# YuemingJin/STswinCL

Measured on AMD Instinct MI355X. Metric: input frames/s, TswinPlus fwd+bwd+Adam, 4-frame 512x512 clips, higher is better.
Workload: dtype bf16; 1 GPU; BASELINE.json configs[1]: TswinPlus(12) seg train step, 4 clips/GPU x T=4 frames x 3x512x512, swin res (64,64), OHEM-CE, Adam; T=4 because the reference asserts it (swin_512.py:313); clips_per_gpu=4, frames_per_clip=4, parallelism=dp1, graph_requested=True

## Files before the change

include/stswin_hip.h:

```cpp
#ifndef STSWIN_HIP_H
#define STSWIN_HIP_H
#ifdef __cplusplus
extern "C" {
#endif

#define STSWIN_GF_GELU 1
#define STSWIN_GF_RESID 2
#define STSWIN_GF_MUL_DGELU 4
#define STSWIN_GF_OUT_F32 8
#define STSWIN_GF_ACCUM 16
#define STSWIN_GF_RELU 32
#define STSWIN_GF_MUL_R 8192
#define STSWIN_GF_C2_DGELU 16384
#define STSWIN_GF_CS_PARTIAL 32768
#define STSWIN_GF_CS_SQ 65536
#define STSWIN_GF_TAPSKIP (1 << 29)
#define STSWIN_GF_BIG 128
#define STSWIN_GF_MID 512
#define STSWIN_GF_NOPIPE 1024
#define STSWIN_GF_HALF 2048
#define STSWIN_GF_M32PP (1u << 31)
#define STSWIN_GF_W4R (1 << 30)
#define STSWIN_GF_ROT 4096
#define STSWIN_GF_NOBIG 256
// ... 33 lines not shown
                        int W, int Ho, int Wo, int C, int backward, void* stream);
int stswin_conv3x3_c64(const void* x, const void* wmat, void* y, const void* resid, float* stats, int frames, int H, int W, int sign,
                       void* stream);
long stswin_conv3x3_c64_wgrad_scratch(int frames, int H, int W);
int stswin_conv3x3_c64_wgrad(const void* dy, const void* x, float* dw, int tapminor, int accumulate, float* scratch, long scratch_floats,
                             int frames, int H, int W, void* stream);

int stswin_gemm_nt(int dtype, const void* A, long lda, const int* a_rows, const void* B, long ldb, void* C, long ldc,
                   const int* c_rows, void* C2, long ldc2, const float* bias, const void* R, long ldr,
                   const int* r_rows, int M, int N, int Kseg, int S, float scale, int scale_cols, int flags,
                   float* colsum , void* stream);
int stswin_cs_reduce(const float* partials, int M, int N, float* out, void* stream);
#define STSWIN_TN_OVERWRITE (1 << 27)
#define STSWIN_TN_NO_COMBINE (1 << 26)
long stswin_gemm_nt_splitk_scratch(int M, int N, int Kseg, int S);
int stswin_gemm_nt_splitk(const void* A, long lda, const int* a_rows, const void* B, long ldb, void* C, long ldc, const float* bias, int M, int N,
                          int Kseg, int S, int relu, float* workspace, long workspace_floats, void* stream);
int stswin_tn_fused_hold(int delta);
int stswin_set_cu_budget(int cus);
int stswin_gemm_tn(int dtype, const void* At, long lda, const int* at_rows, const void* Bt, long ldb, const int* bt_rows,
                   float* C, long ldc, int Mk, int Ni, int Nj, int splits, int bseg,
                   float* workspace , long workspace_floats, void* stream);
#define STSWIN_TN_GROUP_DECLINED (-1050)
typedef struct stswin_tn_problem {
  const void* At; long lda; const int* at_rows;
  const void* Bt; long ldb; const int* bt_rows;
  float* C; long ldc;
  int Mk, Ni, Nj, bseg;
  int overwrite;
  int tapminor;
} stswin_tn_problem;
int stswin_gemm_tn_group(int dtype, int count, const stswin_tn_problem* problems, float* workspace, long workspace_floats, int* splits_out,
                         void* stream);
int stswin_tn_combine(const float* workspace, float* C, long ldc, int Ni, int Nj, int splits, int overwrite, int slab_bf16,
                      void* stream);
#define STSWIN_VAR_F32 100
#define STSWIN_VAR_NT_RING256_REGEPI 1
#define STSWIN_VAR_NT_RING256_LDSEPI 2
#define STSWIN_VAR_NT_RING256_NOPIPE 3
#define STSWIN_VAR_NT_RING256_W4 14
#define STSWIN_VAR_NT_STREAM 4
#define STSWIN_VAR_NT_DUO 5
#define STSWIN_VAR_NT_RING256x128_PP 6
#define STSWIN_VAR_NT_MID 7
#define STSWIN_VAR_NT_256x64 8
#define STSWIN_VAR_NT_128x64 9
#define STSWIN_VAR_NT_128x128 10
#define STSWIN_VAR_NT_128x128_W4 11
#define STSWIN_VAR_NT_SPLITK 13
#define STSWIN_VAR_NT_ROWS 12
#define STSWIN_VAR_TN_RING_PLAIN 20
#define STSWIN_VAR_TN_RING_ATROWS 21
#define STSWIN_VAR_TN_RING_BTROWS 22
#define STSWIN_VAR_TN_RING_BSEG 23
#define STSWIN_VAR_TN_128x128 30
#define STSWIN_VAR_TN_128x128_W4 31
#define STSWIN_VAR_TN_ROWS 32
#define STSWIN_VAR_TN_SLABS_F32 0x1000
#define STSWIN_VAR_TN_SLABS_BF16 0x2000
#define STSWIN_VAR_TN_FUSED 0x8000
#define STSWIN_VAR_TN_TAPMINOR 0x4000
#define STSWIN_TN_OUT_TAPMINOR (1 << 25)
int stswin_gemm_nt_qkv_fp8(const void* A, long lda, const int* a_rows, const void* B, long ldb, void* out8, long ld8, float* scales,
                           long ld_scales, const float* bias, int M, int N, int Kseg, float scale, int scale_cols, int rows_per_problem,
                           int head_dim, void* stream);
int stswin_win_attn_fwd_f8(const void* qkv8, long ld8, const float* scales, long ld_scales, void* out, long ldo, const float* biasT,
// ... 201 lines not shown
```

stswincl_amd/csrc/gemm.hip:

```cpp
#include "common.h"
#include "stswin_hip.h"
#include <cstdint>
#include <cstdlib>
#include <type_traits>

enum {
  GF_GELU = STSWIN_GF_GELU, GF_RESID = STSWIN_GF_RESID, GF_MUL_DGELU = STSWIN_GF_MUL_DGELU, GF_OUT_F32 = STSWIN_GF_OUT_F32,
  GF_ACCUM = STSWIN_GF_ACCUM, GF_RELU = STSWIN_GF_RELU, GF_MUL_R = STSWIN_GF_MUL_R, GF_C2_DGELU = STSWIN_GF_C2_DGELU,
  GF_CS_PARTIAL = STSWIN_GF_CS_PARTIAL, GF_CS_SQ = STSWIN_GF_CS_SQ, GF_TAPSKIP = STSWIN_GF_TAPSKIP,
  GF_WAVES4 = STSWIN_GF_WAVES4, GF_BIG = STSWIN_GF_BIG, GF_NOBIG = STSWIN_GF_NOBIG, GF_MID = STSWIN_GF_MID, GF_NOPIPE = STSWIN_GF_NOPIPE,
  GF_HALF = STSWIN_GF_HALF, GF_ROT = STSWIN_GF_ROT, GF_NOREGEPI = STSWIN_GF_NOREGEPI, GF_NOSTREAM = STSWIN_GF_NOSTREAM,
  GF_DUO = STSWIN_GF_DUO, GF_STREAM = STSWIN_GF_STREAM, GF_NONARROW = STSWIN_GF_NONARROW, GF_NODEEP = STSWIN_GF_NODEEP,
  GF_DEEP = STSWIN_GF_DEEP, GF_W4R = STSWIN_GF_W4R, GF_M32PP = (int)STSWIN_GF_M32PP,
};

#ifdef STSWIN_TUNING
#define STSWIN_DBG(flags, bit) (((flags) & (1 << (bit))) != 0)
#else
#define STSWIN_DBG(flags, bit) false
#endif
enum { GF_DEBUG_BITS = (1 << 17) | (1 << 18) | (1 << 19) | (1 << 20) | (1 << 21) };
#ifdef STSWIN_TUNING
static __device__ int g_dbg_stagger[2] = {8, 0};
extern "C" int stswin_debug_set_stagger(int phases, int ticks) {
// ... 1016 lines not shown
      mma_all();
      if (!lag && kt + 1 < nt) wait_tile(kt + 1);
    }
    if (!lag) __builtin_amdgcn_s_barrier();
    if (arow_bad) __builtin_trap();
    if constexpr (SWAP) epilogue_reg();
    else epilogue();
  }
  if constexpr (PERSIST) {
    tix_ += (int)gridDim.x;
    if (tix_ < ntot_) __syncthreads();
  }
  } while (PERSIST && tix_ < ntot_);
}


#ifdef STSWIN_TUNING
#include "gemm_nt_tuning_kernels.inc"
#endif

struct GemmTN {
  const void* At; long lda; const int* at_rows;
  const void* Bt; long ldb; const int* bt_rows;
  float* C; long ldc;
  int Mk, Ni, Nj;
  int splits;
  int bseg;
  float* slabs;
  int slab_bf16;
  unsigned* tile_cnt; int overwrite; int perm;
};

template <typename T, int NW>
__global__ __launch_bounds__(NW * 64) void gemm_tn_kernel(GemmTN p) {
  constexpr int WN = NW / 2, JN = 128 / WN / 16;
  constexpr int PACK = TT<T>::PACK;
  constexpr int BM = TT<T>::IS_BF16 ? 64 : 32;
  constexpr int ROWB = 128 * sizeof(T);
  constexpr int RPI = 1024 / ROWB;
  constexpr int NI = BM / (NW * RPI);
  constexpr int CPR = ROWB / 16;
  extern __shared__ __attribute__((aligned(16))) char smem[];
  const int tid = threadIdx.x, l = tid & 63, w = wave_id();
  const int wr = w / WN, wc = w % WN;
  const int tiles_j = (p.Nj + 127) >> 7;
  const int split_id = blockIdx.x % p.splits, tile_id = blockIdx.x / p.splits;
  const int i0 = (tile_id / tiles_j) << 7, j0 = (tile_id % tiles_j) << 7;
  const int ntile_all = (p.Mk + BM - 1) / BM;
  const int per = (ntile_all + p.splits - 1) / p.splits;
  const int t_begin = split_id * per, t_end = min(ntile_all, t_begin + per);
  if (t_begin >= t_end) return;

  const char* zero = (const char*)g_stswin_zero;
  const int rsub = l / CPR, cphys = l % CPR;
  long arow[NI], brow[NI];
  int bcol[NI];
  bool btap1[NI];
  const int tap0 = p.bseg > 0 ? j0 / p.bseg : 0;
  const int tap1 = p.bseg > 0 ? min(tap0 + 1, p.Nj / p.bseg - 1) : 0;
#pragma unroll
  for (int i = 0; i < NI; ++i) {
    const int r = (w * NI + i) * RPI + rsub;
    const int cj = j0 + ((cphys & ~15) | ((cphys ^ swz256(r)) & 15)) * PACK;
    bcol[i] = p.bseg > 0 ? cj % p.bseg : cj;
    btap1[i] = p.bseg > 0 && cj / p.bseg != tap0;
  }
  typedef int ivec __attribute__((ext_vector_type(RPI)));
  typedef const __attribute__((address_space(4))) ivec* civec;
  const bool vec_maps = (p.Mk % RPI) == 0;
  auto fetch_rows = [&](int tile) {
    const int mw = tile * BM + w * (NI * RPI);
#pragma unroll
    for (int i = 0; i < NI; ++i) {
      const int mb = mw + i * RPI;
      int va[RPI], vb0[RPI], vb1[RPI];
      if (vec_maps && mb + RPI <= p.Mk) {
        ivec ta, t0, t1;
#pragma unroll
        for (int r = 0; r < RPI; ++r) { ta[r] = mb + r; t0[r] = mb + r; t1[r] = -1; }
// ... 89 lines not shown
          const int col = wr * 64 + i * 16 + fr;
          a[i] = *(const float*)(Ab + row * ROWB + ((((col >> 2) & ~15) | (((col >> 2) ^ swz256(row)) & 15)) << 4) + (col & 3) * 4);
        }
#pragma unroll
        for (int j = 0; j < JN; ++j) {
          const int col = wc * (16 * JN) + j * 16 + fr;
          b[j] = *(const float*)(Bb + row * ROWB + ((((col >> 2) & ~15) | (((col >> 2) ^ swz256(row)) & 15)) << 4) + (col & 3) * 4);
        }
#pragma unroll
        for (int i = 0; i < 4; ++i)
#pragma unroll
          for (int j = 0; j < JN; ++j) acc[i][j] = __builtin_amdgcn_mfma_f32_16x16x4f32(a[i], b[j], acc[i][j], 0, 0, 0);
      }
    }
    if (tk + 2 < t_end) fetch_rows(tk + 2);
  }
#pragma unroll
  for (int i = 0; i < 4; ++i)
#pragma unroll
    for (int j = 0; j < JN; ++j)
#pragma unroll
      for (int r = 0; r < 4; ++r) {
        const int gi = i0 + wr * 64 + i * 16 + 4 * fq + r;
        const int gj = j0 + wc * (16 * JN) + j * 16 + fr;
        if (gi < p.Ni && gj < p.Nj) {
          if (p.slabs) {
            const long so = ((long)split_id * p.Ni + gi) * p.Nj + gj;
            if (p.slab_bf16) ((bf16*)p.slabs)[so] = (bf16)acc[i][j][r];
            else p.slabs[so] = acc[i][j][r];
          }
          else atomicAdd(p.C + (long)gi * p.ldc + gj, acc[i][j][r]);
        }
      }
}


#ifdef STSWIN_TUNING
__device__ unsigned long long* g_tn_stamp_buf = nullptr;
extern "C" int stswin_debug_set_tn_stamps(void* buf) { return (int)hipMemcpyToSymbol(HIP_SYMBOL(g_tn_stamp_buf), &buf, sizeof(buf)); }
#endif
template <int MODE, bool FUSE>
DEVI void gemm_tn_ring_body(const GemmTN& p, const int seq, const int nwg, const int stamp_row) {
  constexpr bool MAPS = MODE != 0, MAP_A = MODE == 1, MAP_B = MODE >= 2, TAPS = MODE == 3;
  using T = bf16;
  constexpr int BMK = 32, ROWB = 512, NST = 4, OP_BYTES = BMK * ROWB, STAGE = 2 * OP_BYTES, PER_STAGE = 4;
  constexpr int FI = 8, FJ = 4;
  extern __shared__ __attribute__((aligned(16))) char smem[];
  const int tid = threadIdx.x, l = tid & 63, w = wave_id();
  const int wr = w >> 2, wc = w & 3;
  const int tiles_j = (p.Nj + 255) >> 8;
  const int ntiles_ = nwg / p.splits;
  const int split_id = seq / ntiles_, tile_id = seq - split_id * ntiles_;
  const int i0 = (tile_id / tiles_j) << 8, j0 = (tile_id % tiles_j) << 8;
  const int nst_all = (p.Mk + BMK - 1) / BMK;
  const int per = (nst_all + p.splits - 1) / p.splits;
  const int s_begin = split_id * per, s_end = min(nst_all, s_begin + per);
  const int nt = max(0, s_end - s_begin);
  const bool dbg_ts = p.ldc == -1;
  auto stamp = [&](int slot) {
    if (dbg_ts && threadIdx.x == 0) ((unsigned long long*)p.C)[(long)stamp_row * 8 + slot] = wall_clock64();
#ifdef STSWIN_TUNING
    else if (g_tn_stamp_buf && threadIdx.x == 0) {
      g_tn_stamp_buf[(long)stamp_row * 8 + slot] = wall_clock64();
      if (slot == 0) { g_tn_stamp_buf[(long)stamp_row * 8 + 6] = (unsigned long long)p.Ni; g_tn_stamp_buf[(long)stamp_row * 8 + 7] = (unsigned long long)(split_id * 1000 + tile_id); }
    }
#endif
// ... 304 lines not shown
__global__ __launch_bounds__(512, 2) void gemm_tn_ring_kernel(GemmTN p) {
  gemm_tn_ring_body<MODE, FUSE>(p, xcd_remap((int)blockIdx.x, (int)gridDim.x), (int)gridDim.x, (int)blockIdx.x);
}

#define TN_GROUP_MAX 4
struct GemmTNGroup { GemmTN q[TN_GROUP_MAX]; int first[TN_GROUP_MAX + 1]; int mode[TN_GROUP_MAX]; int count; };
template <int M0, int M1, int M2, int M3>
__global__ __launch_bounds__(512, 2) void gemm_tn_ring_group_static_kernel(GemmTNGroup g) {
  const int seq = xcd_remap((int)blockIdx.x, (int)gridDim.x);
  if constexpr (M3 >= 0) {
    if (seq >= g.first[3]) { gemm_tn_ring_body<M3 < 0 ? 0 : M3, true>(g.q[3], seq - g.first[3], g.first[4] - g.first[3], (int)blockIdx.x); return; }
  }
  if constexpr (M2 >= 0) {
    if (seq >= g.first[2]) { gemm_tn_ring_body<M2 < 0 ? 0 : M2, true>(g.q[2], seq - g.first[2], g.first[3] - g.first[2], (int)blockIdx.x); return; }
  }
  if constexpr (M1 >= 0) {
    if (seq >= g.first[1]) { gemm_tn_ring_body<M1 < 0 ? 0 : M1, true>(g.q[1], seq - g.first[1], g.first[2] - g.first[1], (int)blockIdx.x); return; }
  }
  gemm_tn_ring_body<M0, true>(g.q[0], seq, g.first[1], (int)blockIdx.x);
}
__global__ __launch_bounds__(512, 2) void gemm_tn_ring_group_kernel(GemmTNGroup g) {
  const int seq = xcd_remap((int)blockIdx.x, (int)gridDim.x);
  int i = 0;
  while (i + 1 < g.count && seq >= g.first[i + 1]) ++i;
  const int local = seq - g.first[i], nwg = g.first[i + 1] - g.first[i];
  switch (g.mode[i]) {
    case 0: gemm_tn_ring_body<0, true>(g.q[i], local, nwg, (int)blockIdx.x); break;
    case 1: gemm_tn_ring_body<1, true>(g.q[i], local, nwg, (int)blockIdx.x); break;
    case 2: gemm_tn_ring_body<2, true>(g.q[i], local, nwg, (int)blockIdx.x); break;
    default: gemm_tn_ring_body<3, true>(g.q[i], local, nwg, (int)blockIdx.x); break;
  }
}

__global__ __launch_bounds__(256) void tn_reduce_kernel(const float* slabs, float* C, long ldc, int Ni, int Nj, int splits,
                                                        int overwrite, int slab_bf16, int perm) {
  if (slab_bf16) {
    const long idx = ((long)blockIdx.x * 256 + threadIdx.x) * 8;
    const long total = (long)Ni * Nj;
    if (idx >= total) return;
    const int i = idx / Nj, j = idx % Nj;
    float a[8] = {0.f, 0.f, 0.f, 0.f, 0.f, 0.f, 0.f, 0.f};
    const bf16* src = (const bf16*)slabs + idx;
    int s = 0;
    for (; s + 8 <= splits; s += 8) {
      bf16x8 v[8];
#pragma unroll
      for (int u = 0; u < 8; ++u) v[u] = *(const bf16x8*)(src + (long)(s + u) * total);
#pragma unroll
      for (int u = 0; u < 8; ++u)
#pragma unroll
        for (int e = 0; e < 8; ++e) a[e] += (float)v[u][e];
    }
    for (; s < splits; ++s) {
      const bf16x8 v = *(const bf16x8*)(src + (long)s * total);
#pragma unroll
      for (int e = 0; e < 8; ++e) a[e] += (float)v[e];
    }
    if (perm > 0) {
      const int S = Nj / perm, sg = j / perm, c = j - sg * perm;
      float* d = C + (long)i * ldc + (long)c * S + sg;
#pragma unroll
      for (int e = 0; e < 8; ++e) d[(long)e * S] = overwrite ? a[e] : d[(long)e * S] + a[e];
      return;
    }
    float* dst = C + (long)i * ldc + j;
    if ((ldc & 3) == 0) {
      f32x4 lo = {a[0], a[1], a[2], a[3]}, hi = {a[4], a[5], a[6], a[7]};
      if (!overwrite) { lo += *(const f32x4*)dst; hi += *(const f32x4*)(dst + 4); }
      *(f32x4*)dst = lo;
      *(f32x4*)(dst + 4) = hi;
    } else {
      for (int e = 0; e < 8; ++e) dst[e] = overwrite ? a[e] : dst[e] + a[e];
    }
    return;
  }
  const long idx = ((long)blockIdx.x * 256 + threadIdx.x) * 4;
  if (idx >= (long)Ni * Nj) return;
  const int i = idx / Nj, j = idx % Nj;
  f32x4 a = {0.f, 0.f, 0.f, 0.f};
  for (int s = 0; s < splits; ++s) a += *(const f32x4*)(slabs + (long)s * Ni * Nj + idx);
  if (perm > 0) {
    const int S = Nj / perm, sg = j / perm, c = j - sg * perm;
    float* d = C + (long)i * ldc + (long)c * S + sg;
#pragma unroll
    for (int e = 0; e < 4; ++e) d[(long)e * S] = overwrite ? a[e] : d[(long)e * S] + a[e];
    return;
  }
  float* dst = C + (long)i * ldc + j;
  if (overwrite) {
    if ((ldc & 3) == 0) *(f32x4*)dst = a;
    else { for (int e = 0; e < 4; ++e) dst[e] = a[e]; }
  } else if ((ldc & 3) == 0) { *(f32x4*)dst = *(const f32x4*)dst + a; }
  else { for (int e = 0; e < 4; ++e) dst[e] += a[e]; }
}

static thread_local int g_last_variant[2] = {0, 0};
extern "C" int stswin_tuning_build() {
#ifdef STSWIN_TUNING
  return 1;
#else
  return 0;
#endif
}
extern "C" int stswin_last_variant(int family) { return family >= 0 && family < 2 ? g_last_variant[family] : -1; }

static int set_lds_once(const void* fn) {
  return (int)hipFuncSetAttribute(fn, hipFuncAttributeMaxDynamicSharedMemorySize, 65536);
}

extern "C" int stswin_cs_reduce(const float* partials, int M, int N, float* out, void* stream) {
  if (M <= 0 || N <= 0) return 0;
  if (N % 4) return -1004;
  const int rows = 2 * ((M + 255) / 256);
  const int rc = stswin_fold_launch(partials, N, 0, rows, N, 1, out, nullptr, nullptr, 0, 1, 1, (hipStream_t)stream);
  if (rc) return rc;
  STSWIN_CHECK_LAUNCH();
  return 0;
}

__global__ __launch_bounds__(256) void gemm_nt_rows_kernel(GemmNT p) {
  const int l = threadIdx.x & 63, n = blockIdx.x * 4 + (threadIdx.x >> 6);
  if (n >= p.N) return;
  const bf16* A = (const bf16*)p.A;
  const bf16* Bn = (const bf16*)p.B + (long)n * p.ldb;
  float acc[8] = {0, 0, 0, 0, 0, 0, 0, 0};
  for (int k = l * 8; k < p.Kseg; k += 512) {
// ... 552 lines not shown
  long wo = 0, to = 0;
  for (int i = 0; i < count; ++i) {
    const StswinTnProblem& q = pr[i];
    const int perm = (q.tapminor && q.bseg > 0) ? q.bseg : 0;
    g.q[i] = GemmTN{q.At, q.lda, q.at_rows, q.Bt, q.ldb, q.bt_rows, q.C, q.ldc, q.Mk, q.Ni, q.Nj, rs[i], q.bseg, workspace + wo, 1,
                    cnt + 3 * to, q.overwrite ? 1 : 0, perm};
    g.mode[i] = q.at_rows ? 1 : (q.bt_rows ? (q.bseg > 0 ? 3 : 2) : 0);
    g.first[i + 1] = g.first[i] + tiles[i] * rs[i];
    wo += ((long)rs[i] * q.Ni * q.Nj + 1) / 2 + 64;
    wo = (wo + 63) / 64 * 64;
    to += tiles[i];
    if (splits_out) splits_out[i] = rs[i];
  }
  for (int i = count; i < TN_GROUP_MAX; ++i) { g.q[i] = g.q[0]; g.mode[i] = 0; g.first[i + 1] = g.first[count]; }
  static int once_g = (int)hipFuncSetAttribute((const void*)gemm_tn_ring_group_kernel, hipFuncAttributeMaxDynamicSharedMemorySize, 131072) |
                      (int)hipFuncSetAttribute((const void*)gemm_tn_ring_group_static_kernel<0, 1, 2, -1>, hipFuncAttributeMaxDynamicSharedMemorySize, 131072) |
                      (int)hipFuncSetAttribute((const void*)gemm_tn_ring_group_static_kernel<0, 0, -1, -1>, hipFuncAttributeMaxDynamicSharedMemorySize, 131072) |
                      (int)hipFuncSetAttribute((const void*)gemm_tn_ring_group_static_kernel<0, 0, 1, 2>, hipFuncAttributeMaxDynamicSharedMemorySize, 131072);
  (void)once_g;
  g_last_variant[1] = STSWIN_VAR_TN_RING_PLAIN | STSWIN_VAR_TN_SLABS_BF16 | STSWIN_VAR_TN_FUSED | (rs[0] << 16);
  const bool m012 = count == 3 && g.mode[0] == 0 && g.mode[1] == 1 && g.mode[2] == 2;
  const bool m00 = count == 2 && g.mode[0] == 0 && g.mode[1] == 0;
  const bool m0012 = count == 4 && g.mode[0] == 0 && g.mode[1] == 0 && g.mode[2] == 1 && g.mode[3] == 2;
  static const char* egd = getenv("STSWIN_TN_GROUP_DYNAMIC");
  if (m012 && !(egd && atoi(egd))) hipLaunchKernelGGL((gemm_tn_ring_group_static_kernel<0, 1, 2, -1>), dim3((unsigned)total), dim3(512), 131072, (hipStream_t)stream, g);
  else if (m00 && !(egd && atoi(egd))) hipLaunchKernelGGL((gemm_tn_ring_group_static_kernel<0, 0, -1, -1>), dim3((unsigned)total), dim3(512), 131072, (hipStream_t)stream, g);
  else if (m0012 && !(egd && atoi(egd))) hipLaunchKernelGGL((gemm_tn_ring_group_static_kernel<0, 0, 1, 2>), dim3((unsigned)total), dim3(512), 131072, (hipStream_t)stream, g);
  else
  hipLaunchKernelGGL(gemm_tn_ring_group_kernel, dim3((unsigned)total), dim3(512), 131072, (hipStream_t)stream, g);
  STSWIN_CHECK_LAUNCH();
  return 0;
}

extern "C" int stswin_gemm_tn(int dtype, const void* At, long lda, const int* at_rows, const void* Bt, long ldb,
                              const int* bt_rows, float* C, long ldc, int Mk, int Ni, int Nj, int splits, int bseg,
                              float* workspace, long workspace_floats, void* stream) {
  if (Mk <= 0 || Ni <= 0 || Nj <= 0) return 0;
  const int overwrite = (splits > 0 && (splits & (1 << 27))) ? 1 : 0;
  const int no_combine = (splits > 0 && (splits & (1 << 26))) ? 1 : 0;
  if (splits > 0) splits &= ~(1 << 26);
  const int perm = (splits > 0 && (splits & (1 << 25)) && bseg > 0 && !no_combine) ? bseg : 0;
  if (splits > 0) splits &= ~(1 << 25);
  const char* f32_env = getenv("STSWIN_TN_F32_SLABS");
  const int f32_slabs = f32_env && atoi(f32_env) ? 1 : 0;
  const int slab_bf16 = (dtype == 0 && !f32_slabs) ? 1 : 0;
  if (splits > 0) splits &= ~(1 << 27);
  const int splits_flags_w4 = (splits > 0 && (splits & (1 << 30))) ? 1 : 0;
  if (splits > 0) splits &= ~(1 << 30);
  const int pack = dtype == 0 ? 8 : 4;
  if (Ni % pack || Nj % pack || lda % pack || ldb % pack) return -1003;
  if (bseg < 0 || (bseg > 0 && (bseg % pack || !bt_rows || Nj % bseg))) return -1004;
  if (dtype == 0 && Mk <= 8 && !at_rows && !bt_rows && bseg == 0 && ldc % 4 == 0) {
    g_last_variant[1] = STSWIN_VAR_TN_ROWS;
    const long nthr = (long)Ni * (Nj / 4);
    hipLaunchKernelGGL(gemm_tn_rows_kernel, dim3((unsigned)((nthr + 255) / 256)), dim3(256), 0, (hipStream_t)stream, (const bf16*)At, lda, (const bf16*)Bt,
                       ldb, C, ldc, Mk, Ni, Nj, overwrite);
    STSWIN_CHECK_LAUNCH();
    return 0;
  }
  if (bseg > 0)
    for (int j0 = 0; j0 < Nj; j0 += 128)
      if ((j0 + 127 < Nj ? j0 + 127 : Nj - 1) / bseg - j0 / bseg > 1) return -1005;
  const int bm = dtype == 0 ? 64 : 32;
  const int ntile = (Mk + bm - 1) / bm;
  const bool force_ring = splits > 0 && (splits & (1 << 29));
  const bool no_ring = splits > 0 && (splits & (1 << 28));
// ... 119 lines not shown
```

stswincl_amd/headops.py:

```python
from __future__ import annotations

import os
import weakref
from typing import List, Optional, Sequence, Tuple

import torch
import torch.nn.functional as F

from . import hip
from .ops import compute_dtype, _f32

KGRAN = 64


_INDEX_MAPS = {}
_TORCH_PADVEC = os.environ.get("STSWIN_TORCH_PADVEC") == "1"
_BN_KEEP_Y = os.environ.get("STSWIN_BN_KEEP_Y") == "1"


class Layout:

    def __init__(self, segs: Sequence[Tuple[int, int, int]], width: int):
        self.segs, self.width = list(segs), width
        self.logical = sum(s[1] for s in self.segs)
# ... 136 lines not shown
        tab = hip.stats_table(Mo, lout.width, x.device) if want_stats else None
        ctx.tapskip = hip.GF_TAPSKIP if (k == 3 and stride == 1 and 2 * dil >= Hin + 3 and Mo <= 32768) else 0
        ctx.halo = (_HALO_CONV and bias is None and lin.is_identity and lout.is_identity and X.is_contiguous()
                    and hip.conv3x3_c64_ok(frames, Hin, Win, lin.width, lout.width, k, stride, pad, dil, dt))
        if ctx.halo:
            hip.conv3x3_c64(X, _conv_mats(weight, dt, lin, lout, False), y, frames, Hin, Win, 1, stats_out=tab)
        else:
            hip.gemm_nt(X, _conv_mats(weight, dt, lin, lout, False), y, M=Mo, a_rows=fmap, S=k * k,
                        bias=lout.pad_vec(bias) if bias is not None else None, stats_out=tab, flags=ctx.tapskip)
        ctx.geom = (frames, Hin, Win)
        ctx.cfg = (k, lin, lout, dt, x.dtype, bias is not None, Mi, Mo)
        ctx.save_for_backward(X, weight, fmap, imap)
        if want_stats:
            ctx.mark_non_differentiable(tab)
            ctx.set_materialize_grads(False)
            return y, tab
        return y

    @staticmethod
    @hip.tn_deferred_backward
    def backward(ctx, dy, _dtab=None):
        if dy is None:
            return (None,) * 8
        X, weight, fmap, imap = ctx.saved_tensors
        k, lin, lout, dt, in_dtype, has_bias, Mi, Mo = ctx.cfg
        co, ci = weight.shape[:2]
        S = k * k
        g = dy.detach().to(dt).contiguous()
        from .ops import wgrad_buffer
        dense = lin.is_identity and lout.is_identity
        direct = dense and S == 1
        dwp = (wgrad_buffer(weight, (lout.width, S * lin.width), X.device) if dense
               else torch.empty(lout.width, S * lin.width, dtype=torch.float32, device=X.device))
        if ctx.halo and _HALO_WGRAD and hip.conv3x3_c64_wgrad_ok(*ctx.geom):
            hip.conv3x3_c64_wgrad(g, X, dwp, *ctx.geom, tapminor=True)
            tapminor = True
        else:
            hip.gemm_tn(g, X, dwp, Mk=Mo, bt_rows=fmap, bseg=lin.width if fmap is not None else 0, overwrite=True,
                        tapminor=dense and S > 1)
            tapminor = dense and S > 1 and hip.last_tn_tapminor()
        dx = None
        if ctx.needs_input_grad[0]:
            dx = torch.empty(Mi, lin.width, dtype=dt, device=X.device)
            pend = ctx.link.take(dt, dx.shape) if ctx.link is not None else None
            if ctx.halo:
                hip.conv3x3_c64(g, _conv_mats(weight, dt, lin, lout, True), dx, *ctx.geom, -1, resid=pend)
            else:
                hip.gemm_nt(g, _conv_mats(weight, dt, lin, lout, True), dx, M=Mi, a_rows=imap, S=S, resid=pend,
                            flags=(hip.GF_RESID if pend is not None else 0) | ctx.tapskip)
            dx = dx.to(in_dtype)
            if ctx.link is not None and not ctx.link.last():
                ctx.link.put(dx)
                dx = None
        hip.tn_join()
        if direct or tapminor:
            dw = dwp
        elif dense:
            dw = dwp.clone().view(co, S, ci).permute(0, 2, 1)
        else:
            dw = torch.zeros(co, ci, S, dtype=torch.float32, device=X.device)
            d3 = dwp.view(lout.width, S, lin.width)
            for oa, on, ob in lout.segs:
                for ia, in_, ib in lin.segs:
                    dw[oa:oa + on, ia:ia + in_, :] = d3[ob:ob + on, :, ib:ib + in_].permute(0, 2, 1)
        db = None
        if has_bias:
            dbp = hip.zeros(lout.width, device=X.device)
            hip.colsum(g, dbp)
            db = lout.unpad_vec(dbp)
# ... 757 lines not shown
```

stswincl_amd/hip.py:

```python
from __future__ import annotations

import ctypes
import functools
import os
import re
from typing import Optional

import torch

_ROOT = os.path.dirname(os.path.dirname(os.path.abspath(__file__)))
LIB_PATH = os.environ.get("STSWIN_HIP_LIB") or os.path.join(_ROOT, "stswincl_amd", "lib", "libstswin_hip.so")
HEADER_PATH = os.path.join(_ROOT, "include", "stswin_hip.h")
_lib: Optional[ctypes.CDLL] = None

_c_int, _c_float, _c_void_p = ctypes.c_int, ctypes.c_float, ctypes.c_void_p


class StswinHipError(RuntimeError):
    pass


_C_TYPES = {"int": ctypes.c_int, "long": ctypes.c_long, "float": ctypes.c_float, "double": ctypes.c_double}


def _c_value(name: str, expr: str) -> int:
    tokens = re.findall(r"0[xX][0-9a-fA-F]+|\d+|<<|[-+*()]|\S", re.sub(r"(?<=[0-9a-fA-F])[uU]\b", "", expr))
    if not tokens or not all(re.fullmatch(r"0[xX][0-9a-fA-F]+|\d+|<<|[-+*()]", t) for t in tokens):
        raise StswinHipError(f"{HEADER_PATH}: cannot evaluate `#define STSWIN_{name} {expr.strip()}`")
    try:
        v = int(eval(" ".join(tokens), {"__builtins__": {}}))
    except (SyntaxError, TypeError) as e:
        raise StswinHipError(f"{HEADER_PATH}: cannot evaluate `#define STSWIN_{name} {expr.strip()}`") from e
    return v - (1 << 32) if v >= 1 << 31 else v


@functools.lru_cache(maxsize=None)
def _header():
    with open(HEADER_PATH) as f:
        text = re.sub(r"/\*.*?\*/", "", f.read(), flags=re.S)
    protos = {}
    for ret, name, params in re.findall(r"\b(int|long)\s+(stswin_\w+)\s*\(([^()]*)\)\s*;", text):
        argtypes = []
        for p in ([] if params.strip() == "void" else params.split(",")):
            words = [w for w in p.split() if w != "const"]
            if "*" in p:
                argtypes.append(ctypes.c_void_p)
            elif len(words) == 2 and words[0] in _C_TYPES:
                argtypes.append(_C_TYPES[words[0]])
            else:
                raise StswinHipError(f"{HEADER_PATH}: {name}: cannot bind parameter `{p.strip()}`")
        protos[name] = (_C_TYPES[ret], argtypes)
    unparsed = set(re.findall(r"\b(stswin_\w+)\s*\(", text)) - set(protos)
    if unparsed:
        raise StswinHipError(f"{HEADER_PATH}: cannot bind the declaration of {sorted(unparsed)}")
    consts = {name: _c_value(name, expr) for name, expr in re.findall(r"^[ \t]*#[ \t]*define[ \t]+STSWIN_(\w+)[ \t]+(\S.*)$", text, flags=re.M)}
    return protos, consts


globals().update(_header()[1])


def declared_symbols():
    return sorted(_header()[0])


def load() -> ctypes.CDLL:
    global _lib
    if _lib is not None:
        return _lib
    if not os.path.exists(LIB_PATH):
        raise StswinHipError(f"{LIB_PATH} not found: run `python __graft_entry__.py` (build()) first; "
                             "stswincl_amd has no CPU or eager fallback")
    lib = ctypes.CDLL(LIB_PATH)
    protos = _header()[0]
    missing = [s for s in sorted(protos) if not hasattr(lib, s)]
    if missing and not os.environ.get("STSWIN_HIP_LIB"):
        raise StswinHipError(f"libstswin_hip.so lacks declared symbols: {missing}")
    for s, (restype, argtypes) in protos.items():
        if s not in missing:
            fn = getattr(lib, s)
            fn.restype, fn.argtypes = restype, argtypes
    _lib = lib
    return lib


def tuning_build() -> bool:
    return bool(load().stswin_tuning_build())

# ... 618 lines not shown
def gemm_tn_group(problems) -> bool:
    n = len(problems)
    if n == 0:
        return True
    first = problems[0]["At"]
    if n > 4 or first.dtype != torch.bfloat16 or torch.cuda.is_current_stream_capturing() and first.device not in _TN_WS:
        return False
    arr = (_TnProblem * n)()
    flops = 0.0
    for i, q in enumerate(problems):
        At, Bt, out = q["At"], q["Bt"], q["out"]
        assert out.dtype == torch.float32 and At.dtype == Bt.dtype == torch.bfloat16
        ar, br = q.get("at_rows"), q.get("bt_rows")
        arr[i] = _TnProblem(At.data_ptr(), _ld(At), ar.data_ptr() if ar is not None else None, Bt.data_ptr(), _ld(Bt),
                            br.data_ptr() if br is not None else None, out.data_ptr(), _ld(out), q["Mk"], out.shape[0], out.shape[1],
                            q.get("bseg", 0), 1 if q.get("overwrite", True) else 0, 1 if q.get("tapminor", False) else 0)
        flops += 2.0 * q["Mk"] * out.shape[0] * out.shape[1]
    ws = _tn_workspace(first.device)
    tn_join()
    sp = (_c_int * n)()
    name = "gemm_tn_bf16"
    if _SHAPE_NAMES:
        name += " group " + " + ".join(f"{q['out'].shape[0]}x{q['out'].shape[1]}" for q in problems) + f" Mk={problems[0]['Mk']}"
    with _Span(name, flops) as span:
        rc = load().stswin_gemm_tn_group(0, n, arr, _p(ws), ws.numel(), sp, _stream())
        if rc == TN_GROUP_DECLINED:
            span.cancel()
    if rc == TN_GROUP_DECLINED:
        return False
    _check(rc, "gemm_tn_group")
    LAST_TN_GROUP_SPLITS[:] = list(sp)
    _log_variant("tn_group", (n, problems[0]["Mk"]) + tuple(sp), 1)
    return True


def last_tn_tapminor() -> bool:
    return bool(load().stswin_last_variant(1) & VAR_TN_TAPMINOR)


def last_variant(family: int) -> dict:
    v = load().stswin_last_variant(family)
    return {"kernel": v & 0xFFF, "slabs": "bf16" if v & VAR_TN_SLABS_BF16 else ("f32" if v & VAR_TN_SLABS_F32 else ""),
            "splits": v >> 16}


def vec_gather(v: torch.Tensor, imap: torch.Tensor, fill: float = 0.0) -> torch.Tensor:
    out = torch.empty(imap.numel(), dtype=torch.float32, device=v.device)
    _check(load().stswin_vec_gather(_p(v), _p(imap), _p(out), imap.numel(), fill, _stream()), "vec_gather")
    return out


def vec_gather_multi(vs, imap: torch.Tensor, fills=None, outs=None):
    k, n = len(vs), imap.numel()
    assert 1 <= k <= 4 and all(v.dtype == torch.float32 and v.is_contiguous() for v in vs)
    if outs is None:
        flat = torch.empty(k, (n + 15) // 16 * 16, dtype=torch.float32, device=imap.device)
        outs = [flat[i, :n] for i in range(k)]
    else:
        assert len(outs) == k and all(o.dtype == torch.float32 and o.is_contiguous() and o.numel() == n for o in outs)
    fills = list(fills) if fills is not None else [0.0] * k
    _check(load().stswin_vec_gather_multi(k, (_c_void_p * k)(*[v.data_ptr() for v in vs]), _p(imap), (_c_void_p * k)(*[o.data_ptr() for o in outs]),
                                          n, (_c_float * k)(*[float(f) for f in fills]), _stream()), "vec_gather_multi")
    return outs


def colsum(y: torch.Tensor, out_f32: torch.Tensor, M: Optional[int] = None):
# ... 1036 lines not shown
```

Before: 630.7 frames/s.

## Defer weight-gradient GEMMs and batch them into one multi-problem split-K launch

Weight-gradient TN GEMMs from the head ops are queued during backward instead of run immediately. They are flushed at the end of the autograd graph task as one grouped kernel covering up to 32 problems, followed by a single combine kernel. A planner picks split-K factors per problem so the total tile count fills the GPU, and orders problems longest-first. This targets launch overhead and poor occupancy from many small wgrad GEMMs, at the cost of deferral bookkeeping, an f32 slab workspace, and checks that each parameter's .grad buffer is unchanged.

```diff
diff --git a/include/stswin_hip.h b/include/stswin_hip.h
--- a/include/stswin_hip.h
+++ b/include/stswin_hip.h
@@ -89,6 +89,14 @@
 } stswin_tn_problem;
 int stswin_gemm_tn_group(int dtype, int count, const stswin_tn_problem* problems, float* workspace, long workspace_floats, int* splits_out,
                          void* stream);
+enum {
+  STSWIN_TN_MULTI_FORCE = 1,
+  STSWIN_TN_MULTI_MAX = 32,
+  STSWIN_VAR_TN_MULTI = 33
+};
+long stswin_gemm_tn_multi_scratch(int count, const stswin_tn_problem* problems);
+int stswin_gemm_tn_multi(int dtype, int count, const stswin_tn_problem* problems, float* workspace, long workspace_floats, int* splits_io,
+                         int flags, void* stream);
 int stswin_tn_combine(const float* workspace, float* C, long ldc, int Ni, int Nj, int splits, int overwrite, int slab_bf16,
                       void* stream);
 #define STSWIN_VAR_F32 100
diff --git a/stswincl_amd/csrc/gemm.hip b/stswincl_amd/csrc/gemm.hip
--- a/stswincl_amd/csrc/gemm.hip
+++ b/stswincl_amd/csrc/gemm.hip
@@ -1072,7 +1072,7 @@
 };
 
 template <typename T, int NW>
-__global__ __launch_bounds__(NW * 64) void gemm_tn_kernel(GemmTN p) {
+__device__ __forceinline__ void gemm_tn_tile_body(const GemmTN& p, const int bid) {
   constexpr int WN = NW / 2, JN = 128 / WN / 16;
   constexpr int PACK = TT<T>::PACK;
   constexpr int BM = TT<T>::IS_BF16 ? 64 : 32;
@@ -1084,7 +1084,7 @@
   const int tid = threadIdx.x, l = tid & 63, w = wave_id();
   const int wr = w / WN, wc = w % WN;
   const int tiles_j = (p.Nj + 127) >> 7;
-  const int split_id = blockIdx.x % p.splits, tile_id = blockIdx.x / p.splits;
+  const int split_id = bid % p.splits, tile_id = bid / p.splits;
   const int i0 = (tile_id / tiles_j) << 7, j0 = (tile_id % tiles_j) << 7;
   const int ntile_all = (p.Mk + BM - 1) / BM;
   const int per = (ntile_all + p.splits - 1) / p.splits;
@@ -1240,6 +1240,31 @@
           else atomicAdd(p.C + (long)gi * p.ldc + gj, acc[i][j][r]);
         }
       }
+}
+template <typename T, int NW>
+__global__ __launch_bounds__(NW * 64) void gemm_tn_kernel(GemmTN p) {
+  gemm_tn_tile_body<T, NW>(p, (int)blockIdx.x);
+}
+
+#define TN_MULTI_MAX 32
+struct TnMultiSlot {
+  const void* At; const int* at_rows; const void* Bt; const int* bt_rows; float* C; float* slabs;
+  int lda, ldb, ldc, Mk, Ni, Nj, splits, bseg, overwrite, perm;
+};
+struct GemmTNMulti {
+  TnMultiSlot q[TN_MULTI_MAX];
+  int first[TN_MULTI_MAX + 1];
+  int cfirst[TN_MULTI_MAX + 1];
+  int count;
+};
+static_assert(sizeof(GemmTNMulti) <= 3584, "the problem table must fit the 4 KB kernel argument beside the hidden arguments");
+__global__ __launch_bounds__(512) void gemm_tn_multi_kernel(GemmTNMulti g) {
+  const int bid = (int)blockIdx.x;
+  int i = 0;
+  while (i + 1 < g.count && bid >= g.first[i + 1]) ++i;
+  const TnMultiSlot& s = g.q[i];
+  const GemmTN p{s.At, s.lda, s.at_rows, s.Bt, s.ldb, s.bt_rows, s.C, s.ldc, s.Mk, s.Ni, s.Nj, s.splits, s.bseg, s.slabs, 0, nullptr, 0, 0};
+  gemm_tn_tile_body<bf16, 8>(p, bid - g.first[i]);
 }
 
 
@@ -1610,6 +1635,34 @@
   }
 }
 
+__device__ __forceinline__ void tn_reduce_f32_body(const float* slabs, float* C, long ldc, int Ni, int Nj, int splits, int overwrite, int perm,
+                                                   long blk) {
+  const long idx = (blk * 256 + threadIdx.x) * 4;
+  if (idx >= (long)Ni * Nj) return;
+  const int i = idx / Nj, j = idx % Nj;
+  f32x4 a = {0.f, 0.f, 0.f, 0.f};
+  for (int s = 0; s < splits; ++s) a += *(const f32x4*)(slabs + (long)s * Ni * Nj + idx);
+  if (perm > 0) {
+    const int S = Nj / perm, sg = j / perm, c = j - sg * perm;
+    float* d = C + (long)i * ldc + (long)c * S + sg;
+#pragma unroll
+    for (int e = 0; e < 4; ++e) d[(long)e * S] = overwrite ? a[e] : d[(long)e * S] + a[e];
+    return;
+  }
+  float* dst = C + (long)i * ldc + j;
+  if (overwrite) {
+    if ((ldc & 3) == 0) *(f32x4*)dst = a;
+    else { for (int e = 0; e < 4; ++e) dst[e] = a[e]; }
+  } else if ((ldc & 3) == 0) { *(f32x4*)dst = *(const f32x4*)dst + a; }
+  else { for (int e = 0; e < 4; ++e) dst[e] += a[e]; }
+}
+__global__ __launch_bounds__(256) void tn_multi_combine_kernel(GemmTNMulti g) {
+  const int bid = (int)blockIdx.x;
+  int i = 0;
+  while (i + 1 < g.count && bid >= g.cfirst[i + 1]) ++i;
+  const TnMultiSlot& s = g.q[i];
+  tn_reduce_f32_body(s.slabs, s.C, s.ldc, s.Ni, s.Nj, s.splits, s.overwrite, s.perm, bid - g.cfirst[i]);
+}
 __global__ __launch_bounds__(256) void tn_reduce_kernel(const float* slabs, float* C, long ldc, int Ni, int Nj, int splits,
                                                         int overwrite, int slab_bf16, int perm) {
   if (slab_bf16) {
@@ -1652,24 +1705,7 @@
     }
     return;
   }
-  const long idx = ((long)blockIdx.x * 256 + threadIdx.x) * 4;
-  if (idx >= (long)Ni * Nj) return;
-  const int i = idx / Nj, j = idx % Nj;
-  f32x4 a = {0.f, 0.f, 0.f, 0.f};
-  for (int s = 0; s < splits; ++s) a += *(const f32x4*)(slabs + (long)s * Ni * Nj + idx);
-  if (perm > 0) {
-    const int S = Nj / perm, sg = j / perm, c = j - sg * perm;
-    float* d = C + (long)i * ldc + (long)c * S + sg;
-#pragma unroll
-    for (int e = 0; e < 4; ++e) d[(long)e * S] = overwrite ? a[e] : d[(long)e * S] + a[e];
-    return;
-  }
-  float* dst = C + (long)i * ldc + j;
-  if (overwrite) {
-    if ((ldc & 3) == 0) *(f32x4*)dst = a;
-    else { for (int e = 0; e < 4; ++e) dst[e] = a[e]; }
-  } else if ((ldc & 3) == 0) { *(f32x4*)dst = *(const f32x4*)dst + a; }
-  else { for (int e = 0; e < 4; ++e) dst[e] += a[e]; }
+  tn_reduce_f32_body(slabs, C, ldc, Ni, Nj, splits, overwrite, perm, (long)blockIdx.x);
 }
 
 static thread_local int g_last_variant[2] = {0, 0};
@@ -2288,6 +2324,88 @@
   return 0;
 }
 
+#include "tn_multi_plan.h"
+static int tn_multi_check(int count, const StswinTnProblem* pr, TnMultiPlanIn* in, const int* forced) {
+  for (int i = 0; i < count; ++i) {
+    const StswinTnProblem& q = pr[i];
+    if (q.Mk <= 0 || q.Ni <= 0 || q.Nj <= 0 || !q.At || !q.Bt || !q.C) return -1052;
+    if (q.Ni % 8 || q.Nj % 8 || q.lda % 8 || q.ldb % 8) return -1003;
+    if (q.bseg < 0 || (q.bseg > 0 && (q.bseg % 8 || !q.bt_rows || q.Nj % q.bseg))) return -1004;
+    if (q.bseg > 0)
+      for (int j0 = 0; j0 < q.Nj; j0 += 128)
+        if ((j0 + 127 < q.Nj ? j0 + 127 : q.Nj - 1) / q.bseg - j0 / q.bseg > 1) return -1005;
+    if (q.tapminor && q.bseg <= 0) return -1052;
+    if (q.lda < 0 || q.ldb < 0 || q.ldc < 0 || q.lda > 0x7FFFFFFFL || q.ldb > 0x7FFFFFFFL || q.ldc > 0x7FFFFFFFL) return -1052;
+    if ((long)q.Ni * q.Nj > 0x7FFFFFFFL) return -1052;
+    in[i].tiles = ((q.Ni + 127) / 128) * ((q.Nj + 127) / 128);
+    in[i].ktiles = (q.Mk + 63) / 64;
+    in[i].out_floats = (long)q.Ni * q.Nj;
+    in[i].forced = forced && forced[i] > 0 ? forced[i] : 0;
+  }
+  return 0;
+}
+extern "C" long stswin_gemm_tn_multi_scratch(int count, const StswinTnProblem* pr) {
+  if (count <= 0) return 0;
+  if (count > TN_MULTI_MAX || !pr) return -1052;
+  TnMultiPlanIn in[TN_MULTI_MAX];
+  const int rc = tn_multi_check(count, pr, in, nullptr);
+  if (rc) return rc;
+  int sp[TN_MULTI_MAX], fill_ok = 0;
+  long need = 0;
+  if (tn_multi_plan(count, in, -1, sp, &need, &fill_ok) < 0) return 0;
+  return need;
+}
+extern "C" int stswin_gemm_tn_multi(int dtype, int count, const StswinTnProblem* pr, float* workspace, long workspace_floats, int* splits_io,
+                                    int flags, void* stream) {
+  if (count <= 0) return 0;
+  if (count > TN_MULTI_MAX || !pr) return -1052;
+  const int declined = STSWIN_TN_GROUP_DECLINED;
+  const bool force = (flags & STSWIN_TN_MULTI_FORCE) != 0;
+  TnMultiPlanIn in[TN_MULTI_MAX];
+  const int rc = tn_multi_check(count, pr, in, force ? splits_io : nullptr);
+  if (rc) return rc;
+  if (dtype != 0 || !workspace || workspace_floats <= 0) return declined;
+  { const char* em = getenv("STSWIN_TN_MULTI"); if (em && atoi(em) == 0 && !force) return declined; }
+  int sp[TN_MULTI_MAX], fill_ok = 0;
+  long need = 0;
+  const long total = tn_multi_plan(count, in, workspace_floats, sp, &need, &fill_ok);
+  if (total < 0 || total > 0x3FFFFFFFL || (!fill_ok && !force)) return declined;
+  int order[TN_MULTI_MAX];
+  for (int i = 0; i < count; ++i) order[i] = i;
+  for (int i = 1; i < count; ++i)
+    for (int k = i; k > 0; --k) {
+      const int a = order[k - 1], b = order[k];
+      if ((in[a].ktiles + sp[a] - 1) / sp[a] >= (in[b].ktiles + sp[b] - 1) / sp[b]) break;
+      order[k - 1] = b; order[k] = a;
+    }
+  GemmTNMulti g;
+  g.count = count;
+  g.first[0] = 0;
+  g.cfirst[0] = 0;
+  long wo = 0;
+  for (int k = 0; k < count; ++k) {
+    const int i = order[k];
+    const StswinTnProblem& q = pr[i];
+    g.q[k] = TnMultiSlot{q.At, q.at_rows, q.Bt, q.bt_rows, q.C, workspace + wo, (int)q.lda, (int)q.ldb, (int)q.ldc, q.Mk, q.Ni, q.Nj, sp[i],
+                         q.bseg, q.overwrite ? 1 : 0, (q.tapminor && q.bseg > 0) ? q.bseg : 0};
+    g.first[k + 1] = g.first[k] + in[i].tiles * sp[i];
+    const long cblocks = (in[i].out_floats / 4 + 255) / 256;
+    if (g.cfirst[k] + cblocks > 0x3FFFFFFFL) return declined;
+    g.cfirst[k + 1] = g.cfirst[k] + (int)cblocks;
+    wo += tn_multi_align((long)sp[i] * in[i].out_floats);
+  }
+  for (int k = count; k < TN_MULTI_MAX; ++k) { g.q[k] = g.q[0]; g.first[k + 1] = g.first[count]; g.cfirst[k + 1] = g.cfirst[count]; }
+  if (splits_io)
+    for (int i = 0; i < count; ++i) splits_io[i] = sp[i];
+  static int once_m = set_lds_once((const void*)gemm_tn_multi_kernel);
+  (void)once_m;
+  g_last_variant[1] = STSWIN_VAR_TN_MULTI | STSWIN_VAR_TN_SLABS_F32 | (sp[0] << 16);
+  hipLaunchKernelGGL(gemm_tn_multi_kernel, dim3((unsigned)g.first[count]), dim3(512), 65536, (hipStream_t)stream, g);
+  hipLaunchKernelGGL(tn_multi_combine_kernel, dim3((unsigned)g.cfirst[count]), dim3(256), 0, (hipStream_t)stream, g);
+  STSWIN_CHECK_LAUNCH();
+  return 0;
+}
+
 extern "C" int stswin_gemm_tn(int dtype, const void* At, long lda, const int* at_rows, const void* Bt, long ldb,
                               const int* bt_rows, float* C, long ldc, int Mk, int Ni, int Nj, int splits, int bseg,
                               float* workspace, long workspace_floats, void* stream) {
diff --git a/stswincl_amd/csrc/tn_multi_plan.h b/stswincl_amd/csrc/tn_multi_plan.h
--- /dev/null
+++ b/stswincl_amd/csrc/tn_multi_plan.h
@@ -0,0 +1,72 @@
+#pragma once
+
+#define TN_MULTI_ROUND 512
+#define TN_MULTI_MIN_KTILES 8
+
+struct TnMultiPlanIn {
+  int tiles, ktiles;
+  long out_floats;
+  int forced;
+};
+
+static inline int tn_multi_no_empty(int ktiles, int splits) {
+  if (splits > ktiles) splits = ktiles;
+  if (splits < 1) splits = 1;
+  const int per = (ktiles + splits - 1) / splits;
+  return (ktiles + per - 1) / per;
+}
+
+static inline int tn_multi_splits_for(int ktiles, long target) {
+  long s = target > 0 ? ktiles / target : 1;
+  if (s < 1) s = 1;
+  if (s > ktiles) s = ktiles;
+  for (int guard = 0; guard < 64 && s > 1; ++guard) {
+    if (s >= 8) s &= ~7L;
+    else { long p2 = 1; while (p2 * 2 <= s) p2 *= 2; s = p2; }
+    const int n = tn_multi_no_empty(ktiles, (int)s);
+    const int per = (ktiles + n - 1) / n;
+    const int last = ktiles - (n - 1) * per;
+    if (n == 1 || (per >= TN_MULTI_MIN_KTILES && last >= TN_MULTI_MIN_KTILES)) return n;
+    s = n < s ? n : s - 1;
+  }
+  return 1;
+}
+
+static inline long tn_multi_align(long floats) { return (floats + 63) / 64 * 64; }
+
+static inline long tn_multi_plan(int count, const TnMultiPlanIn* in, long ws_floats, int* splits, long* ws_need, int* fill_ok) {
+  int kmax = TN_MULTI_MIN_KTILES, any_forced = 0;
+  for (int i = 0; i < count; ++i) {
+    if (in[i].ktiles > kmax) kmax = in[i].ktiles;
+    if (in[i].forced > 0) any_forced = 1;
+  }
+  long best_t = -1;
+  double best_cost = 0.0;
+  for (long t = TN_MULTI_MIN_KTILES; t <= kmax; ++t) {
+    long total = 0, need = 0, load = 0, longest = 0, slab = 0;
+    for (int i = 0; i < count; ++i) {
+      const int s = in[i].forced > 0 ? tn_multi_no_empty(in[i].ktiles, in[i].forced) : tn_multi_splits_for(in[i].ktiles, t);
+      const long per = (in[i].ktiles + s - 1) / s;
+      total += (long)in[i].tiles * s;
+      load += (long)in[i].tiles * s * (per + 2);
+      if (per + 2 > longest) longest = per + 2;
+      slab += (long)s * in[i].out_floats;
+      need += tn_multi_align((long)s * in[i].out_floats);
+    }
+    if (ws_floats >= 0 && need > ws_floats) continue;
+    const double gemm = total <= TN_MULTI_ROUND ? (double)longest : (double)load / TN_MULTI_ROUND + 0.5 * (double)longest;
+    const double cost = gemm + (double)slab / 950e3;
+    if (best_t < 0 || cost < best_cost) { best_t = t; best_cost = cost; }
+    if (any_forced) break;
+  }
+  if (best_t < 0) return -1;
+  long total = 0, need = 0;
+  for (int i = 0; i < count; ++i) {
+    splits[i] = in[i].forced > 0 ? tn_multi_no_empty(in[i].ktiles, in[i].forced) : tn_multi_splits_for(in[i].ktiles, best_t);
+    total += (long)in[i].tiles * splits[i];
+    need += tn_multi_align((long)splits[i] * in[i].out_floats);
+  }
+  *ws_need = need;
+  *fill_ok = total * 2 >= TN_MULTI_ROUND;
+  return total;
+}
diff --git a/stswincl_amd/headops.py b/stswincl_amd/headops.py
--- a/stswincl_amd/headops.py
+++ b/stswincl_amd/headops.py
@@ -192,9 +192,13 @@
         direct = dense and S == 1
         dwp = (wgrad_buffer(weight, (lout.width, S * lin.width), X.device) if dense
                else torch.empty(lout.width, S * lin.width, dtype=torch.float32, device=X.device))
+        hip.wgrad_settle(weight)
         if ctx.halo and _HALO_WGRAD and hip.conv3x3_c64_wgrad_ok(*ctx.geom):
             hip.conv3x3_c64_wgrad(g, X, dwp, *ctx.geom, tapminor=True)
             tapminor = True
+        elif (dense and (S == 1 or fmap is not None) and getattr(weight, "_stswin_grad_dest", None) is None
+              and hip.wgrad_defer(weight, g, X, dwp, Mk=Mo, bt_rows=fmap, bseg=lin.width if fmap is not None else 0, tapminor=S > 1)):
+            tapminor = S > 1
         else:
             hip.gemm_tn(g, X, dwp, Mk=Mo, bt_rows=fmap, bseg=lin.width if fmap is not None else 0, overwrite=True,
                         tapminor=dense and S > 1)
diff --git a/stswincl_amd/hip.py b/stswincl_amd/hip.py
--- a/stswincl_amd/hip.py
+++ b/stswincl_amd/hip.py
@@ -54,6 +54,8 @@
     if unparsed:
         raise StswinHipError(f"{HEADER_PATH}: cannot bind the declaration of {sorted(unparsed)}")
     consts = {name: _c_value(name, expr) for name, expr in re.findall(r"^[ \t]*#[ \t]*define[ \t]+STSWIN_(\w+)[ \t]+(\S.*)$", text, flags=re.M)}
+    for body in re.findall(r"\benum\s*\{([^{}]*)\}", text):
+        consts.update({name: _c_value(name, expr) for name, expr in re.findall(r"\bSTSWIN_(\w+)\s*=\s*([^,]+)", body)})
     return protos, consts
 
 
@@ -738,6 +740,144 @@
     LAST_TN_GROUP_SPLITS[:] = list(sp)
     _log_variant("tn_group", (n, problems[0]["Mk"]) + tuple(sp), 1)
     return True
+
+
+LAST_TN_MULTI_SPLITS: list = []
+
+
+def _tn_problem_array(problems):
+    arr = (_TnProblem * len(problems))()
+    flops = 0.0
+    for i, q in enumerate(problems):
+        At, Bt = q["At"], q["Bt"]
+        assert At.dtype == Bt.dtype
+        ar, br = q.get("at_rows"), q.get("bt_rows")
+        if q.get("out") is not None:
+            out = q["out"]
+            assert out.dtype == torch.float32
+            cptr, ldc, (Ni, Nj) = out.data_ptr(), _ld(out), out.shape
+        else:
+            cptr, ldc, (Ni, Nj) = q["out_ptr"], q["ldc"], q["shape"]
+        arr[i] = _TnProblem(At.data_ptr(), _ld(At), ar.data_ptr() if ar is not None else None, Bt.data_ptr(), _ld(Bt),
+                            br.data_ptr() if br is not None else None, cptr, ldc, q["Mk"], Ni, Nj,
+                            q.get("bseg", 0), 1 if q.get("overwrite", True) else 0, 1 if q.get("tapminor", False) else 0)
+        flops += 2.0 * q["Mk"] * Ni * Nj
+    return arr, flops
+
+
+def gemm_tn_multi(problems, splits=None) -> bool:
+    n = len(problems)
+    if n == 0:
+        return True
+    first = problems[0]["At"]
+    if n > TN_MULTI_MAX:
+        raise StswinHipError(f"gemm_tn_multi: {n} problems, at most {TN_MULTI_MAX} per call")
+    if torch.cuda.is_current_stream_capturing() and first.device not in _TN_WS:
+        return False
+    arr, flops = _tn_problem_array(problems)
+    ws = _tn_workspace(first.device)
+    tn_join()
+    sp = (_c_int * n)(*([int(s) for s in splits] if splits is not None else [0] * n))
+    with _Span("gemm_tn_multi_bf16" + (f" n={n}" if _SHAPE_NAMES else ""), flops) as span:
+        rc = load().stswin_gemm_tn_multi(_dt(first), n, arr, _p(ws), ws.numel(), sp, TN_MULTI_FORCE if splits is not None else 0, _stream())
+        if rc == TN_GROUP_DECLINED:
+            span.cancel()
+    if rc == TN_GROUP_DECLINED:
+        return False
+    _check(rc, "gemm_tn_multi")
+    LAST_TN_MULTI_SPLITS[:] = list(sp)
+    _log_variant("tn_multi", (n,) + tuple(sp), 1)
+    return True
+
+
+_WGRAD_QUEUE: list = []
+_WGRAD_TASK = -1
+
+
+def tn_multi_on() -> bool:
+    return os.environ.get("STSWIN_TN_MULTI") != "0"
+
+
+def tn_multi_wants(Mk: int, Ni: int, Nj: int) -> bool:
+    env = os.environ.get("STSWIN_TN_MULTI_MAX_GFLOP")
+    return 2.0 * Mk * Ni * Nj <= (float(env) if env else 24.0) * 1e9
+
+
+def _param_defers(param) -> bool:
+    if param is None or not isinstance(param, torch.Tensor) or not param.is_leaf or param.grad is not None:
+        return False
+    if param._backward_hooks or getattr(param, "_post_accumulate_grad_hooks", None):
+        return False
+    try:
+        return bool(torch._C._will_engine_execute_node(torch.autograd.graph.get_gradient_edge(param).node))
+    except RuntimeError:
+        return False
+
+
+def wgrad_settle(param) -> bool:
+    if not _WGRAD_QUEUE or torch._C._current_graph_task_id() != _WGRAD_TASK:
+        return False
+    mine = [q for q in _WGRAD_QUEUE if q["param"] is param]
+    if not mine:
+        return False
+    _WGRAD_QUEUE[:] = [q for q in _WGRAD_QUEUE if q["param"] is not param]
+    param._stswin_wgrad_shared = True
+    if not gemm_tn_multi(mine, splits=[0] * len(mine)):
+        raise StswinHipError("deferred weight gradient: the library declined an early flush")
+    return True
+
+
+def wgrad_defer(param, At, Bt, out, *, Mk, at_rows=None, bt_rows=None, bseg=0, tapminor=False) -> bool:
+    Ni, Nj = out.shape
+    if wgrad_settle(param) or getattr(param, "_stswin_wgrad_shared", False):
+        return False
+    if not (tn_multi_on() and At.dtype == torch.bfloat16 and Bt.dtype == torch.bfloat16 and tn_multi_wants(Mk, Ni, Nj)
+            and (bseg == 0 or bseg >= 64) and tn_fused_holds() == 0 and _param_defers(param)):
+        return False
+    if torch.cuda.is_current_stream_capturing() and At.device not in _TN_WS:
+        return False
+    global _WGRAD_TASK
+    task = torch._C._current_graph_task_id()
+    if _WGRAD_QUEUE and task != _WGRAD_TASK:
+        del _WGRAD_QUEUE[:]
+    if not _WGRAD_QUEUE:
+        try:
+            torch.autograd.Variable._execution_engine.queue_callback(wgrad_flush)
+        except RuntimeError:
+            return False
+        _WGRAD_TASK = task
+    _WGRAD_QUEUE.append(dict(At=At, Bt=Bt, at_rows=at_rows, bt_rows=bt_rows, Mk=Mk, bseg=bseg, overwrite=True, tapminor=tapminor,
+                             out_ptr=out.data_ptr(), ldc=_ld(out), shape=(Ni, Nj), param=param))
+    return True
+
+
+def wgrad_pending() -> int:
+    return len(_WGRAD_QUEUE)
+
+
+def wgrad_flush():
+    queue = list(_WGRAD_QUEUE)
+    del _WGRAD_QUEUE[:]
+    for q in queue:
+        g = q["param"].grad
+        if g is None or g.data_ptr() != q["out_ptr"]:
+            raise StswinHipError("deferred weight gradient: the .grad of a parameter of shape "
+                                 f"{tuple(q['param'].shape)} is not the buffer the queued GEMM writes ({'None' if g is None else hex(g.data_ptr())} "
+                                 f"against {hex(q['out_ptr'])}): the gradient was cloned or accumulated before it was written")
+    for a in range(0, len(queue), TN_MULTI_MAX):
+        part = queue[a:a + TN_MULTI_MAX]
+        if gemm_tn_multi(part):
+            continue
+        for q in part:
+            Ni, Nj = q["shape"]
+            out = q["param"].grad.view(-1)[:Ni * Nj].view(Ni, Nj) if q["ldc"] == Nj else None
+            if out is None or out.data_ptr() != q["out_ptr"]:
+                raise StswinHipError("deferred weight gradient: cannot rebuild the output view of a declined problem")
+            gemm_tn(q["At"], q["Bt"], out, Mk=q["Mk"], at_rows=q["at_rows"], bt_rows=q["bt_rows"], bseg=q["bseg"], overwrite=True,
+                    tapminor=q["tapminor"])
+            if q["tapminor"] and q["bseg"] > 0 and not last_tn_tapminor():
+                ci, S = q["bseg"], Nj // q["bseg"]
+                out.view(Ni, ci, S).copy_(out.clone().view(Ni, S, ci).permute(0, 2, 1))
 
 
 def last_tn_tapminor() -> bool:
```

Result: no change. 634.6 frames/s (median of 6 runs) (+0.6%).
